# facebookresearch/habitat-lab

Measured on AMD Instinct MI355X. Metric: env-steps/sec (SPS) PointNav RGB-D 256x256, 64 envs x 128 rollout, higher is better.
Workload: dtype f32; 1 GPU; PointNav SimpleCNN+GRU, 64 envs x 128 steps, 256x256 RGB-D synthetic; envs_per_gpu=64, rollout_steps=128, ppo_epoch=4, num_mini_batch=4, parallelism=dp1

## Files before the change

habitat-lab_amd/csrc/engine.hip:

```cpp
#include <string.h>

#include <algorithm>

#include <string>
#include <vector>

#include "engine.h"

using namespace hab;

static void plan_tm_workspace(hab_policy* e, Arena& wk);
void add_tail_params(hab_policy* e) {
    const hab_policy_desc& d = e->d;
    const int H = d.hidden;
    const std::string rn = "net.state_encoder.rnn.";
    for (int l = 0; l < d.rnn_layers; ++l) {
        const int in = l == 0 ? e->rnn_in : H;
        const std::string sfx = "_l" + std::to_string(l);
        e->i_wih.push_back(add_param(e, rn + "weight_ih" + sfx, {e->G_ * H, in}));
        e->i_whh.push_back(add_param(e, rn + "weight_hh" + sfx, {e->G_ * H, H}));
        e->i_bih.push_back(add_param(e, rn + "bias_ih" + sfx, {e->G_ * H}));
        e->i_bhh.push_back(add_param(e, rn + "bias_hh" + sfx, {e->G_ * H}));
    }
    if (d.action_dist == HAB_DIST_GAUSSIAN) {
// ... 241 lines not shown
}
extern "C" int hab_policy_probe_read_tag(hab_policy* e, int tag, double* total_ms, int* count) {
    if (!e || !total_ms || !count || tag < 0 || tag >= 64) return HAB_ERR_ARG;
    return probe_sum(e, tag, total_ms, count);
}


static int encoder_forward(hab_policy* e, const hab_obs* obs, const uint8_t* masks, const int* rows, int B, hipStream_t s, int f0 = 0, int nB = -1) {
    if (e->rn) { Probe pr(e, HAB_PROBE_ENC_FWD, s); return resnet_encoder_forward(e, obs, masks, rows, B, s, f0, nB); }
    if (nB < 0) nB = B;
    float* W = e->WK;
    float* ws = W + e->w_ws;
    const int H = e->d.hidden;
    if (e->Cin == 0) {
        if (!rows && f0) return HAB_ERR_ARG;
        return gather_cols(obs->goal, e->d.goal_dim, rows ? rows + f0 : nullptr, W + e->w_rnnin + (int64_t)f0 * e->rnn_ld, e->rnn_ld, 0, e->d.goal_dim,
                           e->rnn_ld - e->rnn_in, nB, s);
    }
    const int64_t m1 = (int64_t)e->c1.Ho() * e->c1.Wo() * 32, m2 = (int64_t)e->c2.Ho() * e->c2.Wo() * 64, m3 = e->fc_in;
    float *a1 = W + e->w_a1 + f0 * m1, *a2 = W + e->w_a2 + f0 * m2, *a3 = W + e->w_a3 + f0 * m3, *rin = W + e->w_rnnin + (int64_t)f0 * e->rnn_ld;
    const int* rws = rows ? rows + f0 : nullptr;
    if (!rows && f0) return HAB_ERR_ARG;
    ObsView ov;
    ov.rgb = e->d.has_rgb ? obs->rgb : nullptr; ov.depth = e->d.has_depth ? obs->depth : nullptr; ov.rows = rws;
    ov.H = e->d.H; ov.W = e->d.W; ov.C = e->Cin;
    ConvDesc c1 = e->c1, c2 = e->c2, c3 = e->c3;
    c1.B = c2.B = c3.B = nB;
    { Probe pr(e, HAB_PROBE_CONV1_FWD, s);
      HAB_TRY(obs_conv_fwd(c1, ov, e->PK + e->pk_c1f, e->p(e->i_c1b), a1, 1, ws, e->ws_floats, s, e->pk_c1img >= 0 ? e->PK + e->pk_c1img : nullptr)); }
    { Probe pr(e, HAB_PROBE_CONV2_FWD, s);
      HAB_TRY(conv_fwd(c2, a1, e->PK + e->pk_c2f, e->p(e->i_c2b), a2, 1, ws, e->ws_floats, s)); }
    { Probe pr(e, HAB_PROBE_CONV3_FWD, s);
      HAB_TRY(conv_fwd(c3, a2, e->PK + e->pk_c3f, e->p(e->i_c3b), a3, 0, ws, e->ws_floats, s)); }
    { Probe pr(e, HAB_PROBE_FC_FWD, s);
      HAB_TRY(linear_fwd(a3, e->fc_in, e->PK + e->pk_fc, e->fc_in, e->p(e->i_fcb), rin, e->rnn_ld, nB, H, e->fc_in, 1, 0, ws, e->ws_floats, s)); }
    if (e->d.goal_dim > 0)
        HAB_TRY(gather_cols(obs->goal, e->d.goal_dim, rws, rin, e->rnn_ld, H, e->d.goal_dim, e->rnn_ld - e->rnn_in, nB, s));
    return HAB_OK;
}

static RnnForm rnn_form_cfg(const hab_policy* e, int frames, int n, bool tm_shape) {
    static const int chunks = hab_env_int("HAB_RNN_CHUNKS", 4), chunks_resnet = hab_env_int("HAB_RNN_CHUNKS_RESNET", -1);
    static const int wave = hab_env_int("HAB_RNN_WAVE", 1);
    RnnForm f;
    if (tm_shape) {
        int nc = chunks;
        if (e->rn && chunks > 1) nc = chunks_resnet >= 0 ? chunks_resnet : frames >= 4096 ? 2 : 0;
        f.chunks = std::max(0, std::min(nc, frames / n));
    }
    if (f.chunks == 0) f.wave = wave && e->L >= 2 && e->L <= 4;
    return f;
}
static RnnForm rnn_form(const hab_policy* e, const int* rows, const hab_pack_info* pack, int B, int n) {
    const bool tm_shape = e->Cin > 0 && rows && !pack->env_first_frame && (B % n) == 0 && B / n >= 2 && e->w_ws2 >= 0 &&
                          (int64_t)e->L * 2 * n <= 3 * (int64_t)e->d.max_frames;
    return rnn_form_cfg(e, B, n, tm_shape);
}
static void plan_tm_workspace(hab_policy* e, Arena& wk) {
    const int64_t B = e->d.max_frames;
    if (rnn_form_cfg(e, (int)B, 1, true).chunks == 0) return;
    e->ws2_floats = e->ws_floats;
    e->w_ws2 = wk.take(e->ws2_floats);
    e->w_fmask = wk.take((B + 3) / 4 + 64);
    e->w_iota = wk.take(B + 64);
}
static int tm_setup(hab_policy* e, int nev) {
    if (!e->s2) {
        int lo = 0, hi = 0;
        (void)hipDeviceGetStreamPriorityRange(&lo, &hi);
// ... 430 lines not shown
```

habitat-lab_amd/csrc/gemm_ops.hip:

```cpp
#include "igemm.h"
#include "igemm_dma.h"
#include "igemm_dma_wgrad.h"
#include "igemm_bf3.h"
#include "igemm_bf3_ws.h"
#include "dense_bf3.h"
#include "obs_conv_bf3.h"
#include "obs_conv_bf3_ws.h"
#include "obs_conv_patch.h"
#include "wgrad3x3_bf3.h"
#include "conv2_fwd_strip.h"
#include "conv2_dgrad_strip.h"
#include "obs_wgrad_bf3.h"
#include "conv_patch_bf3.h"
#include "wgrad3x3_patch.h"
#include "prob_build.h"
#include <stdlib.h>

#include <atomic>

#include "../../include/habitat_amd.h"

namespace hab {

static bool no_dma() { static const bool v = hab_env_flag("HAB_NO_DMA"); return v; }
static bool no_merged_dgrad() { static const bool v = hab_env_flag("HAB_NO_MERGED_DGRAD"); return v; }
static bool no_patch() { static const bool v = hab_env_flag("HAB_NO_PATCH"); return v; }
static std::atomic<int> g_bf3_mode{-1};
static int bf3_mode() {
    int m = g_bf3_mode.load(std::memory_order_relaxed);
    if (m < 0) {
        static const int from_env = hab_env_int("HAB_BF3", 2047);
        int expected = -1;
        g_bf3_mode.compare_exchange_strong(expected, from_env, std::memory_order_relaxed);
        m = g_bf3_mode.load(std::memory_order_relaxed);
    }
    return m;
}
int matrix_path_bits() { return bf3_mode(); }
extern "C" int hab_set_matrix_path(int mode) {
    const int prev = bf3_mode();
    if (mode >= 0) g_bf3_mode.store(mode, std::memory_order_relaxed);
    return prev;
}


template <class P, int TM, int TN, int WM, int WN>
static int bf3_launch(const P& p, float* ws, size_t ws_floats, int target_blocks, hipStream_t stream) {
    constexpr bool WS_SHAPE = P::A_RC && P::B_RC && TM == 2 && TN == 2 && WM == 2 && WN == 2;
    if constexpr (WS_SHAPE) {
        constexpr int ws_min_k = 2048;
        if ((bf3_mode() & 32) && p.K >= ws_min_k) return igemm_bf3_ws_launch<P, TM, TN, WM, WN, 4>(p, ws, ws_floats, target_blocks, stream);
    }
    return igemm_bf3_launch<P, TM, TN, WM, WN>(p, ws, ws_floats, target_blocks, stream);
}

template <class P>
static int run_igemm(const P& p, float* ws, size_t ws_floats, hipStream_t stream, int target_blocks = 1024) {
    if (P::A_RC || P::B_RC) target_blocks = 256;
    constexpr bool WG = !P::A_RC && !P::B_RC && AKv<P>::value == 4;
    if constexpr (P::A_RC && P::B_RC) {
        if ((bf3_mode() & 1) && p.M > 64) {
            if (p.N <= 32) return bf3_launch<P, 2, 1, 4, 1>(p, ws, ws_floats, target_blocks, stream);
            if (p.N <= 64) {
                if (p.M >= 256 * 512 && p.K >= 576) return bf3_launch<P, 2, 2, 4, 1>(p, ws, ws_floats, target_blocks, stream);
// ... 43 lines not shown
        return igemm_launch<P, 1, 2, 4, 1>(p, ws, ws_floats, target_blocks, stream);
    } else {
        if (p.M <= 64) return igemm_launch<P, 1, 2, 2, 2>(p, ws, ws_floats, target_blocks, stream);
        return igemm_launch<P, 2, 2, 2, 2>(p, ws, ws_floats, target_blocks, stream);
    }
}

int conv_fwd(const ConvDesc& d, const float* x, const float* wf, const float* bias, float* y, int relu, float* ws,
             size_t ws_floats, hipStream_t stream) {
    ConvFwdProb p;
    HAB_TRY(build(p, d, x, wf, bias, y, relu));
    if ((bf3_mode() & 256) && (bf3_mode() & 1)) {
        const int rc = conv2_fwd_strip(p, ws, ws_floats, stream);
        if (rc != 1) return rc;
    }
    if ((bf3_mode() & 16) && d.stride == 1 && d.KH == 3 && d.KW == 3 && p.M > 64) {
        PatchGeom gq{};
        gq.in = x; gq.Hi = d.H; gq.Wi = d.W; gq.Ci = d.C; gq.Ho = p.g.Ho; gq.Wo = p.g.Wo; gq.KH = 3; gq.KW = 3;
        gq.off_h = -d.pad; gq.off_w = -d.pad; gq.flip = 0;
        const int rc = conv_patch_bf3_dispatch(p, gq, ws, ws_floats, stream);
        if (rc != 1) return rc;
    }
    return run_igemm(p, ws, ws_floats, stream);
}
int64_t obs_conv_weight_image_floats() { return ((int64_t)OCP_W_ELEMS + 1) / 2 + 4; }
int obs_conv_weight_image(const float* wf, int Cout, int KH, int KW, int C, void* img, hipStream_t stream) {
    return obs_conv_patch_weight_image(wf, Cout, KH, KW, C, reinterpret_cast<unsigned short*>(img), stream);
}
int obs_conv_fwd(const ConvDesc& d, const ObsView& obs, const float* wf, const float* bias, float* y, int relu, float* ws,
                 size_t ws_floats, hipStream_t stream, const void* wimg) {
    ObsConvFwdProb p;
    HAB_TRY(build(p, d, obs, wf, bias, y, relu));
    if ((bf3_mode() & 64) && (bf3_mode() & 2) && p.quad) {
        const int rc = obs_conv_patch_launch(p, ws, ws_floats, stream, reinterpret_cast<const unsigned short*>(wimg));
        if (rc != 1) return rc;
    }
    if ((bf3_mode() & 32) && (bf3_mode() & 2) && p.quad && p.M > 64) {
        const int rc = obs_conv_bf3_ws_launch(p, ws, ws_floats, stream);
        if (rc != 1) return rc;
    }
    if ((bf3_mode() & 2) && p.quad && p.M > 64) {
        const int rc = obs_conv_bf3_launch<2>(p, ws, ws_floats, stream);
        if (rc != 1) return rc;
    }
    return run_igemm(p, ws, ws_floats, stream);
}
__global__ void dgrad_empty_class_kernel(ConvDgradProb p) {
    const long long total = (long long)p.g.B * p.Hc * p.Wc * p.N;
    for (long long e = (long long)blockIdx.x * blockDim.x + threadIdx.x; e < total; e += (long long)gridDim.x * blockDim.x)
        p.store((int)(e / p.N), (int)(e % p.N), 0.f);
}

int conv_dgrad(const ConvDesc& d, const float* dy, const float* wd, const float* mask, const float* add, float* dx,
               float* ws, size_t ws_floats, hipStream_t stream) {
    if ((bf3_mode() & 512) && (bf3_mode() & 1)) {
        const int rc = conv2_dgrad_strip(d, dy, wd, mask, add, dx, stream);
        if (rc != 1) return rc;
    }
    if (d.stride > 1 && !no_dma() && !no_merged_dgrad()) {
        ConvDgradMergedProb q;
        HAB_TRY(check_conv(d));
        q.g = make_geom(d);
        if (ConvDgradMergedProb::applicable(q.g)) {
            q.dy = dy; q.w = wd; q.mask = mask; q.add = add; q.dx = dx;
            q.finish();
            if ((bf3_mode() & 1) && q.M > 64) {
                if (q.N <= 32) return bf3_launch<ConvDgradMergedProb, 2, 1, 4, 1>(q, ws, ws_floats, 256, stream);
// ... 42 lines not shown
        ConvWgradProb q = p;
        q.colsum = nullptr;
        if (dbias) HAB_TRY(colsum(dy, p.N, p.K, p.N, dbias, 0, ws, ws_floats, stream));
        return wgrad3x3_patch(q, ws, ws_floats, stream);
    }
    if (ws && d.pad == 0 && p.N <= 32 && !no_dma() && !(bf3_mode() & 8)) {
        ConvWgradProb q = p;
        q.colsum = nullptr;
        if (wgrad_dma_ok(q)) {
            if (dbias) HAB_TRY(colsum(dy, p.N, p.K, p.N, dbias, 0, ws, ws_floats, stream));
            if ((q.M % 288 == 0) || (cdiv(q.M, 288) * 288 < cdiv(q.M, 256) * 256)) return igemm_dma_wgrad_launch<3, 3, 1>(q, ws, ws_floats, 1024, stream);
            return igemm_dma_wgrad_launch<2, 4, 1>(q, ws, ws_floats, 1024, stream);
        }
    }
    return run_igemm(p, ws, ws_floats, stream);
}
int obs_conv_wgrad(const ConvDesc& d, const ObsView& obs, const float* dy, float* dw_oihw, float* dbias, float* ws,
                   size_t ws_floats, hipStream_t stream) {
    ObsConvWgradProb p;
    HAB_TRY(build(p, d, obs, dy, dw_oihw, dbias));
    if ((bf3_mode() & 2) && p.quad && p.K > 4096) {
        const int rc = obs_wgrad_bf3_launch(p, ws, ws_floats, stream);
        if (rc != 1) return rc;
    }
    return run_igemm(p, ws, ws_floats, stream);
}
static bool dense_on() { return (bf3_mode() & 1024) && (bf3_mode() & 1); }
static bool dense_worth(long long M, long long N, long long K) {
    if (bf3_mode() & 2048) return true;
    static const long long min_flop = (long long)hab_env_int("HAB_DENSE_MIN_MFLOP", 4000) * 1000000LL;
    return 2 * M * N * K >= min_flop;
}
int linear_fwd(const float* x, int ldx, const float* w, int ldw, const float* bias, float* y, int ldy, int M, int N, int K,
               int relu, int accumulate, float* ws, size_t ws_floats, hipStream_t stream) {
    LinearFwdProb p;
    HAB_TRY(build(p, x, ldx, w, ldw, bias, y, ldy, M, N, K, relu, accumulate));
    if (dense_on() && dense_worth(M, N, K)) {
        DenseArgs g{};
        g.M = M; g.N = N; g.K = K; g.a = x; g.lda = ldx; g.b = w; g.ldb = ldw; g.c = y; g.ldc = ldy; g.bias = bias; g.relu = relu;
        g.accumulate = accumulate; g.partial = ws;
        g.a_bytes = ((long long)(M - 1) * ldx + K) * 4; g.b_bytes = ((long long)(N - 1) * ldw + K) * 4;
        if (dense_bf3_ok(g, false, false)) {
            g.nsplit = ws ? dense_bf3_splits(g, ws_floats) : 1;
            HAB_TRY((dense_bf3_launch<0, 0>(g, stream)));
            if (g.nsplit > 1) {
                igemm_splitk_reduce<LinearFwdProb>(p, ws, g.nsplit, stream);
                HAB_LAUNCH_CHECK();
            }
            return HAB_OK;
        }
    }
    return run_igemm(p, ws, ws_floats, stream);
}
int linear_dgrad(const float* dy, int lddy, const float* w, int ldw, const float* mask, int ldmask, int mask_cols, float* dx,
                 int lddx, int M, int Nin, int Kout, int accumulate, float* ws, size_t ws_floats, hipStream_t stream) {
    LinearDgradProb p;
    HAB_TRY(build(p, dy, lddy, w, ldw, mask, ldmask, mask_cols, dx, lddx, M, Nin, Kout, accumulate));
    if (dense_on() && !mask && dense_worth(M, Nin, Kout)) {
        DenseArgs g{};
        g.M = M; g.N = Nin; g.K = Kout; g.a = dy; g.lda = lddy; g.b = w; g.ldb = ldw; g.c = dx; g.ldc = lddx; g.accumulate = accumulate;
        g.partial = ws;
        g.a_bytes = ((long long)(M - 1) * lddy + Kout) * 4; g.b_bytes = ((long long)(Kout - 1) * ldw + Nin) * 4;
        if (dense_bf3_ok(g, false, true)) {
            g.nsplit = ws ? dense_bf3_splits(g, ws_floats) : 1;
            HAB_TRY((dense_bf3_launch<0, 1>(g, stream)));
            if (g.nsplit > 1) {
                igemm_splitk_reduce<LinearDgradProb>(p, ws, g.nsplit, stream);
                HAB_LAUNCH_CHECK();
            }
// ... 249 lines not shown
```

habitat-lab_amd/csrc/igemm.h:

```cpp
#pragma once
#include <type_traits>

#include "hab_common.h"

namespace hab {

constexpr int IGEMM_BK = 32;
constexpr int IGEMM_ICPAD = 4;

template <class P, class = void>
struct ColsumB : std::false_type {};
template <class P>
struct ColsumB<P, std::void_t<decltype(P::COLSUM_B)>> : std::bool_constant<P::COLSUM_B && !P::B_RC> {};

template <class P, class = void>
struct AKv : std::integral_constant<int, 4> {};
template <class P>
struct AKv<P, std::void_t<decltype(P::A_KV)>> : std::integral_constant<int, P::A_KV> {};

template <class P, class = void>
struct EpiV4 : std::false_type {};
template <class P>
struct EpiV4<P, std::void_t<decltype(P::EPI_VEC4)>> : std::bool_constant<P::EPI_VEC4> {};

template <class P, int TM, int TN>
__device__ __forceinline__ void igemm_epilogue_v4(const P& p, const f32x16 (&acc)[TM][TN], int mbase, int nbase, int li, int hi) {
    typename P::EpiCol4 ecol[TN][4];
#pragma unroll
    for (int j = 0; j < TN; ++j)
#pragma unroll
        for (int g = 0; g < 4; ++g) ecol[j][g] = p.epi_col4(nbase + j * 32 + 8 * g + 4 * hi);
#pragma unroll
    for (int i = 0; i < TM; ++i) {
        const typename P::EpiRow erow = p.epi_row(mbase + i * 32 + li);
#pragma unroll
        for (int j = 0; j < TN; ++j) {
            typename P::EpiAux4 aux[4];
#pragma unroll
            for (int g = 0; g < 4; ++g) aux[g] = p.epi_fetch4(erow, ecol[j][g]);
#pragma unroll
            for (int g = 0; g < 4; ++g) {
                f32x4 v;
                v[0] = acc[i][j][4 * g]; v[1] = acc[i][j][4 * g + 1]; v[2] = acc[i][j][4 * g + 2]; v[3] = acc[i][j][4 * g + 3];
                p.epi_store4(erow, ecol[j][g], aux[g], v);
            }
        }
    }
}

template <class P, int TM, int TN>
__device__ __forceinline__ void igemm_partial_v4(const P& p, const f32x16 (&acc)[TM][TN], float* __restrict__ slab, int mbase, int nbase,
                                                 int li, int hi) {
    const bool vec = ((p.N & 3) == 0) && ((reinterpret_cast<uintptr_t>(slab) & 15) == 0);
#pragma unroll
    for (int i = 0; i < TM; ++i) {
        const int row = mbase + i * 32 + li;
// ... 234 lines not shown
#pragma unroll
        for (int g = 0; g < 4; ++g) {
            typename P::EpiRow erow[4];
            typename P::EpiAux eaux[4][TN];
#pragma unroll
            for (int q = 0; q < 4; ++q) {
                erow[q] = p.epi_row(m0 + (wm * TM + i) * 32 + q + 8 * g + 4 * hi);
#pragma unroll
                for (int j = 0; j < TN; ++j) eaux[q][j] = p.epi_fetch(erow[q], ecol[j]);
            }
#pragma unroll
            for (int q = 0; q < 4; ++q)
#pragma unroll
                for (int j = 0; j < TN; ++j) p.epi_store(erow[q], ecol[j], eaux[q][j], acc[i][j][g * 4 + q]);
        }
}

template <class P, bool WIDE>
__global__ void __launch_bounds__(256) igemm_splitk_reduce_kernel(const P p, const float* __restrict__ partial, int splits) {
    __shared__ float red[4][64];
    int MP = p.M;
    if constexpr (ColsumB<P>::value) MP += (p.colsum != nullptr) ? 1 : 0;
    const size_t total = (size_t)MP * p.N;
    if constexpr (!WIDE) {
        for (size_t e = (size_t)blockIdx.x * 256 + threadIdx.x; e < total; e += (size_t)gridDim.x * 256) {
            float s = 0.0f;
            for (int z = 0; z < splits; ++z) s += partial[(size_t)z * total + e];
            const int m = (int)(e / p.N), n = (int)(e % p.N);
            if constexpr (ColsumB<P>::value) {
                if (m == p.M) { p.store_colsum(n, s); continue; }
            }
            p.store(m, n, s);
        }
        return;
    }
    const int tx = threadIdx.x & 63, ty = threadIdx.x >> 6;
    const int chunk = (splits + 3) >> 2;
    const int z0 = ty * chunk, z1 = min(splits, z0 + chunk);
    for (size_t e0 = (size_t)blockIdx.x * 64; e0 < total; e0 += (size_t)gridDim.x * 64) {
        const size_t e = e0 + tx;
        float s = 0.0f;
        if (e < total) {
            const float* src = partial + e;
            int z = z0;
            for (; z + 8 <= z1; z += 8) {
                float v[8];
#pragma unroll
                for (int u = 0; u < 8; ++u) v[u] = src[(size_t)(z + u) * total];
#pragma unroll
                for (int u = 0; u < 8; ++u) s += v[u];
            }
            for (; z < z1; ++z) s += src[(size_t)z * total];
        }
        red[ty][tx] = s;
        __syncthreads();
        if (ty == 0 && e < total) {
            s = (red[0][tx] + red[1][tx]) + (red[2][tx] + red[3][tx]);
            const int m = (int)(e / p.N), n = (int)(e % p.N);
            bool done = false;
            if constexpr (ColsumB<P>::value) {
                if (m == p.M) { p.store_colsum(n, s); done = true; }
            }
            if (!done) p.store(m, n, s);
        }
        __syncthreads();
    }
}

template <class P>
inline void igemm_splitk_reduce(const P& p, const float* ws, int splits, hipStream_t stream) {
    const long long total = (long long)(p.M + 1) * p.N;
    if (splits >= 16) {
        int blocks = (int)cdivl(total, 64);
        if (blocks > 8192) blocks = 8192;
        igemm_splitk_reduce_kernel<P, true><<<blocks, 256, 0, stream>>>(p, ws, splits);
    } else {
        int blocks = (int)cdivl(total, 256);
        if (blocks > 4096) blocks = 4096;
        igemm_splitk_reduce_kernel<P, false><<<blocks, 256, 0, stream>>>(p, ws, splits);
    }
}

struct IgemmPlan {
    int splits = 1;
    int k_per_split = 0;
    size_t partial_floats = 0;
};

inline IgemmPlan igemm_plan(int BM, int BN, int M, int N, int K, int target_blocks, int max_splits, size_t max_partial_floats) {
    IgemmPlan pl;
    const long long tiles = (long long)cdiv(M, BM) * cdiv(N, BN);
    int splits = 1;
    if (tiles < target_blocks) splits = (int)((target_blocks + tiles - 1) / tiles);
    const int ktiles = cdiv(K, IGEMM_BK);
    if (splits > ktiles) splits = ktiles;
    if (splits > max_splits) splits = max_splits;
    while (splits > 1 && (size_t)splits * (size_t)(M + 1) * (size_t)N > max_partial_floats) --splits;
    if (splits < 1) splits = 1;
    pl.k_per_split = cdiv(ktiles, splits) * IGEMM_BK;
    pl.splits = cdiv(K, pl.k_per_split);
    pl.partial_floats = pl.splits > 1 ? (size_t)pl.splits * (M + 1) * N : 0;
    return pl;
}

// ... 20 lines not shown
```

habitat-lab_amd/csrc/obs_conv_patch.h:

```cpp
#pragma once
#include <utility>

#include "igemm_bf3.h"

namespace hab {

constexpr int OCP_TH = 4;
constexpr int OCP_R = 4 * OCP_TH + 4;
constexpr int OCP_KP = 256 + 8;
constexpr int OCP_DP = 64 + 8;

constexpr int OCP_W_ELEMS = 3 * 32 * OCP_KP + 2 * 32 * OCP_DP;
__global__ void obs_patch_split_weights(const float* __restrict__ w, int N, unsigned short* __restrict__ img) {
    const int e = blockIdx.x * blockDim.x + threadIdx.x;
    if (e >= 32 * 256) return;
    const int n = e >> 8, k = e & 255, c = k & 3;
    float v = n < N ? w[(size_t)n * 256 + k] : 0.f;
    if (c < 3) v *= HAB_RCP255;
    unsigned h1, h2, h3;
    bf3_split(v, h1, h2, h3);
    img[(0 * 32 + n) * OCP_KP + k] = (unsigned short)h1;
    img[(1 * 32 + n) * OCP_KP + k] = (unsigned short)h2;
    img[(2 * 32 + n) * OCP_KP + k] = (unsigned short)h3;
    if (c == 3) {
        unsigned short* d = img + 3 * 32 * OCP_KP;
        const int kd = k >> 2;
        d[(0 * 32 + n) * OCP_DP + kd] = (unsigned short)h1;
        d[(1 * 32 + n) * OCP_DP + kd] = (unsigned short)h2;
    }
    if (k < 8) {
        img[(0 * 32 + n) * OCP_KP + 256 + k] = 0; img[(1 * 32 + n) * OCP_KP + 256 + k] = 0; img[(2 * 32 + n) * OCP_KP + 256 + k] = 0;
        unsigned short* d = img + 3 * 32 * OCP_KP;
        d[(0 * 32 + n) * OCP_DP + 64 + k] = 0; d[(1 * 32 + n) * OCP_DP + 64 + k] = 0;
    }
}

template <class F, int... Is>
__device__ __forceinline__ void ocp_static_for_impl(F& f, std::integer_sequence<int, Is...>) { (f(std::integral_constant<int, Is>()), ...); }
template <int N, class F>
__device__ __forceinline__ void ocp_static_for(F& f) { ocp_static_for_impl(f, std::make_integer_sequence<int, N>()); }

struct ObsPatchGeom {
    int W, H, Ho, Wo, tiles_per_img, ntiles;
    int units;
    int patch_elems;
};

template <int UPT>
__global__ void __launch_bounds__(512) obs_conv_patch_kernel(const ObsConvFwdProb p, const ObsPatchGeom gq, const unsigned short* __restrict__ wimg,
                                                              const int sign_schedule, const int ablate) {
    using P = ObsConvFwdProb;
    static_assert(EpiV4<P>::value, "transposed-accumulator epilogue");
    extern __shared__ __attribute__((aligned(16))) unsigned short smem16[];
    const int W = gq.W;
    const int t = threadIdx.x;
    const int lane = t & 63, wave = __builtin_amdgcn_readfirstlane(t >> 6), group = wave >> 2, gw = wave & 3, tg = t & 255;
    const int li = lane & 31, hi = lane >> 5;
    unsigned short* W12 = smem16;
    unsigned short* WD1 = W12 + 2 * 32 * OCP_KP;
    float* biasL = reinterpret_cast<float*>(WD1 + 32 * OCP_DP);
    unsigned short* P0 = WD1 + 32 * OCP_DP + 64 + group * gq.patch_elems;
    unsigned short* P1 = P0 + OCP_R * W * 4;
    unsigned short* P2 = P1 + OCP_R * W;

    for (int i = t; i < 2 * 32 * OCP_KP / 8; i += 512) reinterpret_cast<u32x4*>(W12)[i] = reinterpret_cast<const u32x4*>(wimg)[i];
    for (int i = t; i < 32 * OCP_DP / 8; i += 512) reinterpret_cast<u32x4*>(WD1)[i] = reinterpret_cast<const u32x4*>(wimg + 3 * 32 * OCP_KP)[i];
    if (t < 32) biasL[t] = (p.bias && t < p.N) ? p.bias[t] : 0.f;
    bf16x8 w3f[8][2], wd2f[4];
    {
        const unsigned short* w3 = wimg + 2 * 32 * OCP_KP + li * OCP_KP + hi * 8;
        const unsigned short* wd = wimg + 3 * 32 * OCP_KP + li * OCP_DP + hi * 8;
#pragma unroll
        for (int kh = 0; kh < 8; ++kh)
#pragma unroll
            for (int s = 0; s < 2; ++s) w3f[kh][s] = *reinterpret_cast<const bf16x8*>(w3 + kh * 32 + s * 16);
#pragma unroll
        for (int j = 0; j < 4; ++j) wd2f[j] = *reinterpret_cast<const bf16x8*>(wd + 32 * OCP_DP + j * 16);
    }

    auto tile_of = [&](int vb) {
        const int q = gq.ntiles >> 3, r = gq.ntiles & 7, xcd = vb & 7, idx = vb >> 3;
// ... 10 lines not shown
        return (size_t)p.obs.srow(img) * gq.H;
    };
    auto unit_pix = [&](size_t frame, int y0, int j, bool& ok) {
        const int u = tg + 256 * j;
        const int r = u / qpr, x4 = u - r * qpr;
        const int y = y0 + r;
        ok = (u < gq.units) & (y < gq.H);
        return (frame + (ok ? y : 0)) * W + 4 * (ok ? x4 : 0);
    };
    auto fetch_depth = [&](int tile) {
        if (ablate & 1) return;
        int y0;
        const size_t frame = tile_base(tile, y0);
#pragma unroll
        for (int j = 0; j < UPT; ++j) {
            bool ok;
            const size_t pix = unit_pix(frame, y0, j, ok);
            dp[j] = ld4(p.obs.depth + pix);
            if (!ok) dp[j] = zero4();
        }
    };
    auto fetch_rgb = [&](int tile) {
        if (ablate & 1) return;
        int y0;
        const size_t frame = tile_base(tile, y0);
#pragma unroll
        for (int j = 0; j < UPT; ++j) {
            bool ok;
            const size_t pix = unit_pix(frame, y0, j, ok);
            rg[j] = *reinterpret_cast<const Rgb12*>(p.obs.rgb + pix * 3);
            if (!ok) { rg[j].d0 = 0; rg[j].d1 = 0; rg[j].d2 = 0; }
        }
    };
    auto stage = [&]() {
        if (ablate & 8) return;
#pragma unroll
        for (int j = 0; j < UPT; ++j) {
            const int u = tg + 256 * j;
            if (u >= gq.units) continue;
            const unsigned d[3] = {rg[j].d0, rg[j].d1, rg[j].d2};
            unsigned f[12];
#pragma unroll
            for (int e = 0; e < 12; ++e) f[e] = __float_as_uint((float)((d[e >> 2] >> (8 * (e & 3))) & 0xffu));
            unsigned a1, a2, a3, b1, b2, b3;
            bf3_split2(dp[j][0], dp[j][1], a1, a2, a3);
            bf3_split2(dp[j][2], dp[j][3], b1, b2, b3);
            u32x4 lo, hi4;
            lo[0] = bf3_pack(f[0], f[1]);  lo[1] = bf3_pack(f[2], a1 << 16);
            lo[2] = bf3_pack(f[3], f[4]);  lo[3] = bf3_pack(f[5], a1 & 0xffff0000u);
            hi4[0] = bf3_pack(f[6], f[7]); hi4[1] = bf3_pack(f[8], b1 << 16);
            hi4[2] = bf3_pack(f[9], f[10]); hi4[3] = bf3_pack(f[11], b1 & 0xffff0000u);
            unsigned short* dst = P0 + (size_t)u * 16;
            *reinterpret_cast<u32x4*>(dst) = lo;
            *reinterpret_cast<u32x4*>(dst + 8) = hi4;
            u32x2 r1, r2;
            r1[0] = a2; r1[1] = b2; r2[0] = a3; r2[1] = b3;
            *reinterpret_cast<u32x2*>(P1 + (size_t)u * 4) = r1;
            *reinterpret_cast<u32x2*>(P2 + (size_t)u * 4) = r2;
        }
    };

    const int a_px0 = (4 * gw) * W + 4 * li;
    f32x16 acc[2];
    bf16x8 fr[2][5];
    auto load_step = [&](auto stc) {
        constexpr int st = decltype(stc)::value, set = st & 1;
        if constexpr (st < 4) {
#pragma unroll
            for (int i = 0; i < 2; ++i) {
                const int px = a_px0 + (2 * st + hi) * W + 128 * i;
                u32x4 v1, v2;
                const u32x2 l1 = *reinterpret_cast<const u32x2*>(P1 + px), h1 = *reinterpret_cast<const u32x2*>(P1 + px + 4);
                const u32x2 l2 = *reinterpret_cast<const u32x2*>(P2 + px), h2 = *reinterpret_cast<const u32x2*>(P2 + px + 4);
                v1[0] = l1[0]; v1[1] = l1[1]; v1[2] = h1[0]; v1[3] = h1[1];
                v2[0] = l2[0]; v2[1] = l2[1]; v2[2] = h2[0]; v2[3] = h2[1];
                fr[set][i] = __builtin_bit_cast(bf16x8, v1);
                fr[set][2 + i] = __builtin_bit_cast(bf16x8, v2);
            }
            fr[set][4] = *reinterpret_cast<const bf16x8*>(WD1 + li * OCP_DP + (2 * st + hi) * 8);
        } else {
            constexpr int kh = (st - 4) >> 1, s_ = (st - 4) & 1;
#pragma unroll
            for (int i = 0; i < 2; ++i)
                fr[set][i] = *reinterpret_cast<const bf16x8*>(P0 + (size_t)(a_px0 + kh * W + 128 * i) * 4 + (2 * s_ + hi) * 8);
#pragma unroll
            for (int pl = 0; pl < 2; ++pl)
                fr[set][2 + pl] = *reinterpret_cast<const bf16x8*>(W12 + (pl * 32 + li) * OCP_KP + kh * 32 + s_ * 16 + hi * 8);
        }
    };
    auto flip = [&](bf16x8 f, const unsigned sgn) {
        u32x4 v = __builtin_bit_cast(u32x4, f);
        v[0] ^= sgn; v[1] ^= sgn; v[2] ^= sgn; v[3] ^= sgn;
        return __builtin_bit_cast(bf16x8, v);
    };
    auto mma_step = [&](auto stc, const unsigned sgn) {
        constexpr int st = decltype(stc)::value, set = st & 1;
        if constexpr (st < 4) {
            const bf16x8 a1[2] = {flip(fr[set][0], sgn), flip(fr[set][1], sgn)}, a2[2] = {flip(fr[set][2], sgn), flip(fr[set][3], sgn)};
            const bf16x8 wd1 = fr[set][4];
#pragma unroll
            for (int i = 0; i < 2; ++i) acc[i] = __builtin_amdgcn_mfma_f32_32x32x16_bf16(wd1, a2[i], acc[i], 0, 0, 0);
#pragma unroll
            for (int i = 0; i < 2; ++i) acc[i] = __builtin_amdgcn_mfma_f32_32x32x16_bf16(wd2f[st], a1[i], acc[i], 0, 0, 0);
#pragma unroll
            for (int i = 0; i < 2; ++i) acc[i] = __builtin_amdgcn_mfma_f32_32x32x16_bf16(wd1, a1[i], acc[i], 0, 0, 0);
        } else {
            constexpr int kh = (st - 4) >> 1, s_ = (st - 4) & 1;
            const bf16x8 a[2] = {flip(fr[set][0], sgn), flip(fr[set][1], sgn)};
#pragma unroll
            for (int i = 0; i < 2; ++i) acc[i] = __builtin_amdgcn_mfma_f32_32x32x16_bf16(w3f[kh][s_], a[i], acc[i], 0, 0, 0);
#pragma unroll
            for (int i = 0; i < 2; ++i) acc[i] = __builtin_amdgcn_mfma_f32_32x32x16_bf16(fr[set][3], a[i], acc[i], 0, 0, 0);
#pragma unroll
            for (int i = 0; i < 2; ++i) acc[i] = __builtin_amdgcn_mfma_f32_32x32x16_bf16(fr[set][2], a[i], acc[i], 0, 0, 0);
        }
    };
    auto matrix_phase = [&](const unsigned sgn) {
#pragma unroll
        for (int i = 0; i < 2; ++i)
#pragma unroll
            for (int v = 0; v < 16; ++v) acc[i][v] = 0.0f;
        if (ablate & 2) return;
        load_step(std::integral_constant<int, 0>());
// ... 3 lines not shown
            mma_step(stc, sgn);
        };
        ocp_static_for<20>(body);
    };
    auto store_tile = [&](int tile, bool neg) {
        if ((ablate & 4) && acc[0][0] != 12345.f) return;
        const int img = tile / gq.tiles_per_img, ho = (tile - img * gq.tiles_per_img) * OCP_TH + gw;
        if (ho >= gq.Ho) return;
#pragma unroll
        for (int i = 0; i < 2; ++i) {
            const int wo = 32 * i + li;
            if (wo >= gq.Wo) continue;
            const size_t base = ((size_t)(img * gq.Ho + ho) * gq.Wo + wo) * p.N;
#pragma unroll
            for (int g = 0; g < 4; ++g) {
                const int n = 8 * g + 4 * hi;
                if (n + 3 >= p.N) continue;
                f32x4 v;
                v[0] = acc[i][4 * g]; v[1] = acc[i][4 * g + 1]; v[2] = acc[i][4 * g + 2]; v[3] = acc[i][4 * g + 3];
                if (neg) { v[0] = -v[0]; v[1] = -v[1]; v[2] = -v[2]; v[3] = -v[3]; }
                v += *reinterpret_cast<const f32x4*>(biasL + n);
                if (p.relu) { v[0] = fmaxf(v[0], 0.f); v[1] = fmaxf(v[1], 0.f); v[2] = fmaxf(v[2], 0.f); v[3] = fmaxf(v[3], 0.f); }
                if (p.y) *reinterpret_cast<f32x4*>(p.y + base + n) = v;
            }
        }
    };

    const int vstep = 2 * gridDim.x;
    const int vb0 = blockIdx.x + group * gridDim.x;
    const int n_mine = vb0 < gq.ntiles ? (gq.ntiles - vb0 + vstep - 1) / vstep : 0;
    const int n_first = (int)blockIdx.x < gq.ntiles ? (gq.ntiles - (int)blockIdx.x + vstep - 1) / vstep : 0;
    if (n_first == 0) return;
    if (n_mine > 0) { fetch_depth(tile_of(vb0)); if (group == 0) fetch_rgb(tile_of(vb0)); }
    if (group == 0) stage();
    __syncthreads();
    for (int pI = 0; pI <= 2 * n_first; ++pI) {
        if ((pI & 1) == group) {
            const int k = pI >> 1;
            if (k < n_mine) {
                if (k + 1 < n_mine) fetch_depth(tile_of(vb0 + (k + 1) * vstep));
                const int tile = tile_of(vb0 + k * vstep);
                matrix_phase((sign_schedule && (tile & 1)) ? 0x80008000u : 0u);
            }
        } else {
            const int kd = (pI - 1 - group) / 2;
            const int ks = (pI + 1 - group) / 2;
            if (ks < n_mine) {
                fetch_rgb(tile_of(vb0 + ks * vstep));
                stage();
            }
            if (pI >= 1 + group && kd < n_mine) {
                const int tile_d = tile_of(vb0 + kd * vstep);
                store_tile(tile_d, sign_schedule && (tile_d & 1));
            }
        }
        __syncthreads();
    }
}

inline int obs_conv_patch_weight_image(const float* w_packed, int N, int KH, int KW, int C, unsigned short* img, hipStream_t stream) {
    if (KH != 8 || KW != 8 || C != 4 || N > 32 || (N & 3) || !w_packed || !img || (reinterpret_cast<uintptr_t>(img) & 15)) return 1;
    obs_patch_split_weights<<<32, 256, 0, stream>>>(w_packed, N, img);
    HAB_LAUNCH_CHECK();
    return HAB_OK;
}

inline int obs_conv_patch_launch(const ObsConvFwdProb& p, float* ws, size_t ws_floats, hipStream_t stream, const unsigned short* wimg_cached = nullptr) {
    const ConvGeom& g = p.g;
    if (!p.quad || g.KH != 8 || g.KW != 8 || g.stride != 4 || g.pad != 0 || p.N > 32 || (p.N & 3) || p.K != 256 || g.W > 256 || (g.W & 3) || g.Wo > 64 ||
        g.Wo < 1 || p.M <= 0)
        return 1;
    if (!wimg_cached && (!ws || ws_floats * 4 < (size_t)OCP_W_ELEMS * 2 || (reinterpret_cast<uintptr_t>(ws) & 15))) return 1;
    if (reinterpret_cast<uintptr_t>(wimg_cached) & 15) return 1;
    ObsPatchGeom gq;
    gq.W = g.W; gq.H = g.H; gq.Ho = g.Ho; gq.Wo = g.Wo;
    gq.tiles_per_img = cdiv(g.Ho, OCP_TH);
    gq.ntiles = g.B * gq.tiles_per_img;
    gq.units = OCP_R * (g.W >> 2);
    if (cdiv(gq.units, 256) > 5) return 1;
    gq.patch_elems = OCP_R * g.W * 6 + 64;
    const size_t lds = ((size_t)2 * 32 * OCP_KP + 32 * OCP_DP + 64 + (size_t)2 * gq.patch_elems) * 2;
    if (lds > 160 * 1024) return 1;
    const unsigned short* wimg = wimg_cached;
    if (!wimg) {
        unsigned short* built = reinterpret_cast<unsigned short*>(ws);
        obs_patch_split_weights<<<32, 256, 0, stream>>>(p.w, p.N, built);
        HAB_LAUNCH_CHECK();
        wimg = built;
    }
    auto kern = obs_conv_patch_kernel<5>;
    static const hipError_t attr_err = hipFuncSetAttribute(reinterpret_cast<const void*>(kern), hipFuncAttributeMaxDynamicSharedMemorySize, 160 * 1024);
    if (attr_err != hipSuccess) return (int)attr_err;
    static const int sign_schedule = !hab_env_flag("HAB_BF3_NOSIGN");
    static const int ablate = hab_env_int("HAB_OCP_ABLATE", 0);
    const int pairs = (gq.ntiles + 1) / 2;
    const int grid = pairs < 256 ? (pairs + 7) / 8 * 8 : 256;
    kern<<<grid, 512, lds, stream>>>(p, gq, wimg, sign_schedule, ablate);
    HAB_LAUNCH_CHECK();
    return HAB_OK;
}

}
```

habitat-lab_amd/csrc/ops.h:

```cpp
#pragma once
#include "hab_common.h"

namespace hab {

struct ConvDesc {
    int B, H, W, C, Cout, KH, KW, stride, pad;
    int Creal = 0;
    int Ho() const { return (H + 2 * pad - KH) / stride + 1; }
    int Wo() const { return (W + 2 * pad - KW) / stride + 1; }
};
struct ObsView;

int conv_fwd(const ConvDesc& d, const float* x, const float* wf, const float* bias, float* y, int relu, float* ws,
             size_t ws_floats, hipStream_t stream);
int obs_conv_fwd(const ConvDesc& d, const ObsView& obs, const float* wf, const float* bias, float* y, int relu, float* ws,
                 size_t ws_floats, hipStream_t stream, const void* wimg = nullptr);
int64_t obs_conv_weight_image_floats();
int obs_conv_weight_image(const float* wf, int Cout, int KH, int KW, int C, void* img, hipStream_t stream);
int conv_dgrad(const ConvDesc& d, const float* dy, const float* wd, const float* mask, const float* add, float* dx,
               float* ws, size_t ws_floats, hipStream_t stream);
int conv_wgrad(const ConvDesc& d, const float* x, const float* dy, float* dw_oihw, float* dbias, float* ws, size_t ws_floats,
               hipStream_t stream);
int obs_conv_wgrad(const ConvDesc& d, const ObsView& obs, const float* dy, float* dw_oihw, float* dbias, float* ws,
                   size_t ws_floats, hipStream_t stream);
int linear_fwd(const float* x, int ldx, const float* w, int ldw, const float* bias, float* y, int ldy, int M, int N, int K,
               int relu, int accumulate, float* ws, size_t ws_floats, hipStream_t stream);
int linear_dgrad(const float* dy, int lddy, const float* w, int ldw, const float* mask, int ldmask, int mask_cols, float* dx,
                 int lddx, int M, int Nin, int Kout, int accumulate, float* ws, size_t ws_floats, hipStream_t stream);
int linear_wgrad(const float* dy, int lddy, const float* x, int ldx, float* dw, int lddw, int Mrows, int Nout, int Kin,
                 int perm_c, int perm_hw, int accumulate, float* ws, size_t ws_floats, hipStream_t stream);
int colsum(const float* a, int lda, int M, int N, float* out, int accumulate, float* ws, size_t ws_floats, hipStream_t stream);
int repack_conv(const float* w_oihw, float* wf, float* wd, int Cout, int Cin, int KH, int KW, int cpad, hipStream_t stream);
int repack_flatten(const float* w, float* wp, int N, int C, int HW, hipStream_t stream);
int transpose2d(const float* w, float* wt, int R, int C, hipStream_t stream);
int pad_rows(const float* w, float* wp, int R, int C, int ld, hipStream_t stream);

struct PackInfo {
    const int* select_inds;
    const int* step_offsets;
    const int* num_seqs_at_step;
    const int* frag_env;
    const int* frag_start;
    int P, F, max_len, n_envs;
};

struct RnnLayerParams {
    const float* w_ih; const float* w_hh; const float* b_ih; const float* b_hh;
    const float* w_hh_t;
    float* dw_ih; float* dw_hh; float* db_ih; float* db_hh;
    int in_dim;
    const float* w_ih_pad = nullptr;
    int w_ih_ld = 0;
};

struct RnnWork {
    float* gi;
    float* gates;
    float* hn;
    float* hprev;
// ... 39 lines not shown
```

habitat-lab_amd/csrc/prob_build.h:

```cpp
#pragma once
#include "ops.h"
#include "problems.h"

namespace hab {

inline ConvGeom make_geom(const ConvDesc& d) {
    ConvGeom g;
    g.B = d.B; g.H = d.H; g.W = d.W; g.C = d.C; g.Cout = d.Cout; g.KH = d.KH; g.KW = d.KW; g.stride = d.stride; g.pad = d.pad;
    g.finish();
    return g;
}

inline int check_conv(const ConvDesc& d) {
    if (d.B <= 0 || d.H <= 0 || d.W <= 0 || d.C <= 0 || d.Cout <= 0 || d.KH <= 0 || d.KW <= 0 || d.stride <= 0 || d.pad < 0)
        return HAB_ERR_ARG;
    if ((long long)d.B * d.H * d.W >= (1ll << 31)) return HAB_ERR_UNSUPPORTED;
    if ((d.H + 2 * d.pad - d.KH) < 0 || (d.W + 2 * d.pad - d.KW) < 0) return HAB_ERR_ARG;
    return HAB_OK;
}

inline bool aligned16(const void* p) { return (((uintptr_t)p) & 15) == 0; }

inline int obs_quad_ok(const ConvDesc& d, const ObsView& obs) {
    return obs.rgb && obs.depth && obs.C == 4 && d.KW % 4 == 0 && d.stride % 4 == 0 && d.pad == 0 && d.W % 4 == 0 &&
// ... 19 lines not shown
}
inline int build(ConvDgradProb& p, const ConvDesc& d, const float* dy, const float* wd, const float* mask, const float* add,
                 float* dx, int ph = 0, int pw = 0) {
    HAB_TRY(check_conv(d));
    if (d.C % 4 || d.Cout % 4) return HAB_ERR_UNSUPPORTED;
    if (ph < 0 || pw < 0 || ph >= d.stride || pw >= d.stride) return HAB_ERR_ARG;
    p.g = make_geom(d);
    p.dy = dy; p.w = wd; p.mask = mask; p.add = add; p.dx = dx;
    p.set_class(ph, pw);
    return HAB_OK;
}
inline int build(ConvWgradProb& p, const ConvDesc& d, const float* x, const float* dy, float* dw, float* dbias = nullptr) {
    HAB_TRY(check_conv(d));
    if (d.C % 4 || d.Cout % 4) return HAB_ERR_UNSUPPORTED;
    p.g = make_geom(d);
    p.M = d.KH * d.KW * d.C; p.N = d.Cout; p.K = d.B * p.g.Ho * p.g.Wo;
    p.x = x; p.dy = dy; p.dw = dw; p.colsum = dbias;
    p.Creal = d.Creal > 0 ? d.Creal : d.C;
    return HAB_OK;
}
inline int build(ObsConvWgradProb& p, const ConvDesc& d, const ObsView& obs, const float* dy, float* dw, float* dbias = nullptr) {
    HAB_TRY(check_conv(d));
    if (d.C != obs.C || d.Cout % 4) return HAB_ERR_UNSUPPORTED;
    p.g = make_geom(d);
    p.M = d.KH * d.KW * d.C; p.N = d.Cout; p.K = d.B * p.g.Ho * p.g.Wo;
    p.obs = obs; p.dy = dy; p.dw = dw; p.colsum = dbias;
    p.quad = obs_quad_ok(d, obs);
    return HAB_OK;
}
inline int build(LinearFwdProb& p, const float* x, int ldx, const float* w, int ldw, const float* bias, float* y, int ldy,
                 int M, int N, int K, int relu, int accumulate) {
    if (M <= 0 || N <= 0 || K <= 0 || !x || !w || !y) return HAB_ERR_ARG;
    p.M = M; p.N = N; p.K = K; p.x = x; p.ldx = ldx; p.w = w; p.ldw = ldw; p.bias = bias; p.y = y; p.ldy = ldy;
    p.relu = relu; p.accumulate = accumulate;
    p.vec = (ldx % 4 == 0 && ldw % 4 == 0 && K % 4 == 0 && aligned16(x) && aligned16(w)) ? 1 : 0;
    return HAB_OK;
}
inline int build(LinearDgradProb& p, const float* dy, int lddy, const float* w, int ldw, const float* mask, int ldmask,
                 int mask_cols, float* dx, int lddx, int M, int Nin, int Kout, int accumulate) {
    if (M <= 0 || Nin <= 0 || Kout <= 0 || !dy || !w || !dx) return HAB_ERR_ARG;
    if (!aligned16(w)) return HAB_ERR_ARG;
    p.M = M; p.N = Nin; p.K = Kout; p.dy = dy; p.lddy = lddy; p.w = w; p.ldw = ldw; p.mask = mask; p.ldmask = ldmask;
    p.mask_cols = mask_cols; p.dx = dx; p.lddx = lddx; p.accumulate = accumulate;
    p.vec_a = (lddy % 4 == 0 && Kout % 4 == 0 && aligned16(dy)) ? 1 : 0;
    return HAB_OK;
}
inline int build(LinearWgradProb& p, const float* dy, int lddy, const float* x, int ldx, float* dw, int lddw, int Mrows,
                 int Nout, int Kin, int perm_c, int perm_hw, int accumulate) {
    if (Mrows <= 0 || Nout <= 0 || Kin <= 0 || !dy || !x || !dw) return HAB_ERR_ARG;
    if (!aligned16(dy) || !aligned16(x)) return HAB_ERR_ARG;
    p.M = Nout; p.N = Kin; p.K = Mrows; p.dy = dy; p.lddy = lddy; p.x = x; p.ldx = ldx; p.dw = dw; p.lddw = lddw;
    p.perm_c = perm_c; p.perm_hw = perm_hw; p.dPermC = FastDiv(perm_c > 0 ? perm_c : 1); p.accumulate = accumulate;
    return HAB_OK;
}

}
```

habitat-lab_amd/csrc/problems.h:

```cpp
#pragma once
#include <math.h>

#include "hab_common.h"
#include "bf3_split.h"

namespace hab {

#define HAB_HD __host__ __device__ inline

HAB_HD f32x4 zero4() {
    f32x4 z;
    z[0] = 0.f; z[1] = 0.f; z[2] = 0.f; z[3] = 0.f;
    return z;
}
HAB_HD f32x4 ld4(const float* p) { return *reinterpret_cast<const f32x4*>(p); }

struct Raw4 { f32x4 v; int ok; };
struct KKey { int k, ok; };
HAB_HD KKey kkey(int k, int k_end) { KKey q; q.k = k; q.ok = k < k_end; return q; }
HAB_HD f32x4 sel4(const Raw4& r) { return r.ok ? r.v : zero4(); }
struct NoCtx {};
struct NoAux {};

constexpr int HAB_FAR = -(1 << 28);
// ... 874 lines not shown
        if (!(r.ok & c.ok)) return;
        dw[(size_t)c.n * g.C * g.KH * g.KW + r.off] = v * r.scale;
    }
    HAB_GENERIC_STORE
};

HAB_HD Raw4 row_fetch4(const float* row, int row_ok, const KKey& q, int K, int vec) {
    Raw4 r;
    if (vec) {
        r.ok = row_ok & q.ok;
        r.v = ld4(row + (q.k & -r.ok));
    } else {
        r.ok = 1;
        r.v = zero4();
        for (int e = 0; e < 4; ++e)
            if (row_ok && q.ok && q.k + e < K) r.v[e] = row[q.k + e];
    }
    return r;
}
HAB_HD Raw4 col_fetch4(const float* base, int ld, int r, int r_ok, int j, int n) {
    Raw4 q;
    if (((ld & 3) == 0) && (j + 3 < n || j >= n)) {
        q.ok = r_ok & (j < n);
        q.v = ld4(base + (((size_t)r * ld + j) & (size_t)(-(long long)q.ok)));
    } else {
        q.ok = 1;
        q.v = zero4();
        for (int e = 0; e < 4; ++e)
            if (r_ok && j + e < n) q.v[e] = base[(size_t)r * ld + j + e];
    }
    return q;
}

struct LinearFwdProb {
    static constexpr bool A_RC = true, B_RC = true;
    int M, N, K;
    const float* x; int ldx;
    const float* w; int ldw;
    const float* bias;
    float* y; int ldy;
    int relu, vec;
    int accumulate;
    HAB_NO_KCTX
    using ACtx = WRowCtx;
    using BCtx = WRowCtx;
    using ARaw = Raw4;
    using BRaw = Raw4;
    HAB_HD ACtx a_ctx(int m) const { ACtx c; c.ok = m < M; c.row = c.ok ? x + (size_t)m * ldx : x; return c; }
    using AKey = KKey;
    using BKey = KKey;
    HAB_HD AKey a_key(const KCtx&, int k, int k_end) const { return kkey(k, k_end); }
    HAB_HD BKey b_key(const KCtx&, int k, int k_end) const { return kkey(k, k_end); }
    HAB_HD ARaw a_fetch(const ACtx& c, const KCtx&, const AKey& q) const { return row_fetch4(c.row, c.ok, q, K, vec); }
    HAB_HD BCtx b_ctx(int n) const { BCtx c; c.ok = n < N; c.row = c.ok ? w + (size_t)n * ldw : w; return c; }
    HAB_HD BRaw b_fetch(const BCtx& c, const KCtx&, const BKey& q) const { return row_fetch4(c.row, c.ok, q, K, vec); }
    HAB_PLAIN_CVT
    using EpiCol = ColN;
    using EpiRow = RowBase;
    struct EpiAux { float old; };
    HAB_HD EpiCol epi_col(int n) const { EpiCol c; c.n = n; c.ok = n < N; c.bias = (bias && c.ok) ? bias[n] : 0.f; return c; }
    HAB_HD EpiRow epi_row(int m) const { EpiRow r; r.ok = m < M; r.base = (size_t)m * ldy; return r; }
    HAB_HD EpiAux epi_fetch(const EpiRow& r, const EpiCol& c) const {
        EpiAux a;
        a.old = accumulate ? y[(r.ok & c.ok) ? r.base + c.n : 0] : 0.f;
        return a;
    }
    HAB_HD void epi_store(const EpiRow& r, const EpiCol& c, const EpiAux& a, float v) const {
        if (!(r.ok & c.ok)) return;
        v += c.bias;
        v += a.old;
        if (relu) v = v > 0.f ? v : 0.f;
        y[r.base + c.n] = v;
    }
    HAB_GENERIC_STORE
};
// ... 98 lines not shown
```

Measured before the change: 62990 env-steps/s.

## Fuse goal-column gather into FC split-K reduce and pre-sign staged obs patches

The goal-vector gather into the RNN input buffer is folded into the split-K reduce epilogue of the FC linear forward, which removes a separate gather_cols launch whenever that path runs. Separately, the obs conv1 patch kernel gets a template variant that applies the alternating-tile sign flip while staging to LDS rather than on every fragment in the matrix phase. Both are enabled by default through new HAB_BF3 bits. The tail write only fires on the split-K path and otherwise falls back to the old gather via a host-side written flag, and it adds a strided scalar loop to the reduce kernel.

```diff
diff --git a/habitat-lab_amd/csrc/engine.hip b/habitat-lab_amd/csrc/engine.hip
--- a/habitat-lab_amd/csrc/engine.hip
+++ b/habitat-lab_amd/csrc/engine.hip
@@ -297,9 +297,14 @@
       HAB_TRY(conv_fwd(c2, a1, e->PK + e->pk_c2f, e->p(e->i_c2b), a2, 1, ws, e->ws_floats, s)); }
     { Probe pr(e, HAB_PROBE_CONV3_FWD, s);
       HAB_TRY(conv_fwd(c3, a2, e->PK + e->pk_c3f, e->p(e->i_c3b), a3, 0, ws, e->ws_floats, s)); }
+    int goal_written = 0;
+    ColsTail goal;
+    goal.src = obs->goal; goal.src_ld = e->d.goal_dim; goal.rows = rws; goal.col0 = H; goal.ncols = e->d.goal_dim; goal.npad = e->rnn_ld - e->rnn_in;
+    goal.written = &goal_written;
     { Probe pr(e, HAB_PROBE_FC_FWD, s);
-      HAB_TRY(linear_fwd(a3, e->fc_in, e->PK + e->pk_fc, e->fc_in, e->p(e->i_fcb), rin, e->rnn_ld, nB, H, e->fc_in, 1, 0, ws, e->ws_floats, s)); }
-    if (e->d.goal_dim > 0)
+      HAB_TRY(linear_fwd(a3, e->fc_in, e->PK + e->pk_fc, e->fc_in, e->p(e->i_fcb), rin, e->rnn_ld, nB, H, e->fc_in, 1, 0, ws, e->ws_floats, s,
+                         (e->d.goal_dim > 0 && obs->goal) ? &goal : nullptr)); }
+    if (e->d.goal_dim > 0 && !goal_written)
         HAB_TRY(gather_cols(obs->goal, e->d.goal_dim, rws, rin, e->rnn_ld, H, e->d.goal_dim, e->rnn_ld - e->rnn_in, nB, s));
     return HAB_OK;
 }
diff --git a/habitat-lab_amd/csrc/gemm_ops.hip b/habitat-lab_amd/csrc/gemm_ops.hip
--- a/habitat-lab_amd/csrc/gemm_ops.hip
+++ b/habitat-lab_amd/csrc/gemm_ops.hip
@@ -29,7 +29,7 @@
 static int bf3_mode() {
     int m = g_bf3_mode.load(std::memory_order_relaxed);
     if (m < 0) {
-        static const int from_env = hab_env_int("HAB_BF3", 2047);
+        static const int from_env = hab_env_int("HAB_BF3", 2047 | 8192 | 16384);
         int expected = -1;
         g_bf3_mode.compare_exchange_strong(expected, from_env, std::memory_order_relaxed);
         m = g_bf3_mode.load(std::memory_order_relaxed);
@@ -139,7 +139,7 @@
     ObsConvFwdProb p;
     HAB_TRY(build(p, d, obs, wf, bias, y, relu));
     if ((bf3_mode() & 64) && (bf3_mode() & 2) && p.quad) {
-        const int rc = obs_conv_patch_launch(p, ws, ws_floats, stream, reinterpret_cast<const unsigned short*>(wimg));
+        const int rc = obs_conv_patch_launch(p, ws, ws_floats, stream, reinterpret_cast<const unsigned short*>(wimg), (bf3_mode() & 16384) != 0);
         if (rc != 1) return rc;
     }
     if ((bf3_mode() & 32) && (bf3_mode() & 2) && p.quad && p.M > 64) {
@@ -248,9 +248,10 @@
     return 2 * M * N * K >= min_flop;
 }
 int linear_fwd(const float* x, int ldx, const float* w, int ldw, const float* bias, float* y, int ldy, int M, int N, int K,
-               int relu, int accumulate, float* ws, size_t ws_floats, hipStream_t stream) {
+               int relu, int accumulate, float* ws, size_t ws_floats, hipStream_t stream, const ColsTail* tail) {
     LinearFwdProb p;
     HAB_TRY(build(p, x, ldx, w, ldw, bias, y, ldy, M, N, K, relu, accumulate));
+    if (tail && (bf3_mode() & 8192)) p.tail = *tail;
     if (dense_on() && dense_worth(M, N, K)) {
         DenseArgs g{};
         g.M = M; g.N = N; g.K = K; g.a = x; g.lda = ldx; g.b = w; g.ldb = ldw; g.c = y; g.ldc = ldy; g.bias = bias; g.relu = relu;
diff --git a/habitat-lab_amd/csrc/igemm.h b/habitat-lab_amd/csrc/igemm.h
--- a/habitat-lab_amd/csrc/igemm.h
+++ b/habitat-lab_amd/csrc/igemm.h
@@ -22,6 +22,11 @@
 struct EpiV4 : std::false_type {};
 template <class P>
 struct EpiV4<P, std::void_t<decltype(P::EPI_VEC4)>> : std::bool_constant<P::EPI_VEC4> {};
+
+template <class P, class = void>
+struct SplitkTail : std::false_type {};
+template <class P>
+struct SplitkTail<P, std::void_t<decltype(P::SPLITK_TAIL)>> : std::bool_constant<P::SPLITK_TAIL> {};
 
 template <class P, int TM, int TN>
 __device__ __forceinline__ void igemm_epilogue_v4(const P& p, const f32x16 (&acc)[TM][TN], int mbase, int nbase, int li, int hi) {
@@ -322,6 +327,7 @@
             }
             p.store(m, n, s);
         }
+        if constexpr (SplitkTail<P>::value) p.store_tail((int)(blockIdx.x * 256 + threadIdx.x), (int)(gridDim.x * 256));
         return;
     }
     const int tx = threadIdx.x & 63, ty = threadIdx.x >> 6;
@@ -355,11 +361,15 @@
         }
         __syncthreads();
     }
+    if constexpr (SplitkTail<P>::value) p.store_tail((int)(blockIdx.x * 256 + threadIdx.x), (int)(gridDim.x * 256));
 }
 
 template <class P>
 inline void igemm_splitk_reduce(const P& p, const float* ws, int splits, hipStream_t stream) {
     const long long total = (long long)(p.M + 1) * p.N;
+    if constexpr (SplitkTail<P>::value) {
+        if (p.tail.src && p.tail.written) *p.tail.written = 1;
+    }
     if (splits >= 16) {
         int blocks = (int)cdivl(total, 64);
         if (blocks > 8192) blocks = 8192;
diff --git a/habitat-lab_amd/csrc/obs_conv_patch.h b/habitat-lab_amd/csrc/obs_conv_patch.h
--- a/habitat-lab_amd/csrc/obs_conv_patch.h
+++ b/habitat-lab_amd/csrc/obs_conv_patch.h
@@ -46,7 +46,7 @@
     int patch_elems;
 };
 
-template <int UPT>
+template <int UPT, bool STAGE_SIGN>
 __global__ void __launch_bounds__(512) obs_conv_patch_kernel(const ObsConvFwdProb p, const ObsPatchGeom gq, const unsigned short* __restrict__ wimg,
                                                               const int sign_schedule, const int ablate) {
     using P = ObsConvFwdProb;
@@ -123,7 +123,7 @@
             if (!ok) { rg[j].d0 = 0; rg[j].d1 = 0; rg[j].d2 = 0; }
         }
     };
-    auto stage = [&]() {
+    auto stage = [&](const unsigned sgn) {
         if (ablate & 8) return;
 #pragma unroll
         for (int j = 0; j < UPT; ++j) {
@@ -141,11 +141,16 @@
             lo[2] = bf3_pack(f[3], f[4]);  lo[3] = bf3_pack(f[5], a1 & 0xffff0000u);
             hi4[0] = bf3_pack(f[6], f[7]); hi4[1] = bf3_pack(f[8], b1 << 16);
             hi4[2] = bf3_pack(f[9], f[10]); hi4[3] = bf3_pack(f[11], b1 & 0xffff0000u);
+            u32x2 r1, r2;
+            r1[0] = a2; r1[1] = b2; r2[0] = a3; r2[1] = b3;
+            if constexpr (STAGE_SIGN) {
+#pragma unroll
+                for (int q = 0; q < 4; ++q) { lo[q] ^= sgn; hi4[q] ^= sgn; }
+                r1[0] ^= sgn; r1[1] ^= sgn; r2[0] ^= sgn; r2[1] ^= sgn;
+            }
             unsigned short* dst = P0 + (size_t)u * 16;
             *reinterpret_cast<u32x4*>(dst) = lo;
             *reinterpret_cast<u32x4*>(dst + 8) = hi4;
-            u32x2 r1, r2;
-            r1[0] = a2; r1[1] = b2; r2[0] = a3; r2[1] = b3;
             *reinterpret_cast<u32x2*>(P1 + (size_t)u * 4) = r1;
             *reinterpret_cast<u32x2*>(P2 + (size_t)u * 4) = r2;
         }
@@ -180,6 +185,7 @@
         }
     };
     auto flip = [&](bf16x8 f, const unsigned sgn) {
+        if constexpr (STAGE_SIGN) return f;
         u32x4 v = __builtin_bit_cast(u32x4, f);
         v[0] ^= sgn; v[1] ^= sgn; v[2] ^= sgn; v[3] ^= sgn;
         return __builtin_bit_cast(bf16x8, v);
@@ -249,7 +255,8 @@
     const int n_first = (int)blockIdx.x < gq.ntiles ? (gq.ntiles - (int)blockIdx.x + vstep - 1) / vstep : 0;
     if (n_first == 0) return;
     if (n_mine > 0) { fetch_depth(tile_of(vb0)); if (group == 0) fetch_rgb(tile_of(vb0)); }
-    if (group == 0) stage();
+    auto tile_sgn = [&](int tile) { return (sign_schedule && (tile & 1)) ? 0x80008000u : 0u; };
+    if (group == 0) stage(n_mine > 0 ? tile_sgn(tile_of(vb0)) : 0u);
     __syncthreads();
     for (int pI = 0; pI <= 2 * n_first; ++pI) {
         if ((pI & 1) == group) {
@@ -257,14 +264,15 @@
             if (k < n_mine) {
                 if (k + 1 < n_mine) fetch_depth(tile_of(vb0 + (k + 1) * vstep));
                 const int tile = tile_of(vb0 + k * vstep);
-                matrix_phase((sign_schedule && (tile & 1)) ? 0x80008000u : 0u);
+                matrix_phase(tile_sgn(tile));
             }
         } else {
             const int kd = (pI - 1 - group) / 2;
             const int ks = (pI + 1 - group) / 2;
             if (ks < n_mine) {
-                fetch_rgb(tile_of(vb0 + ks * vstep));
-                stage();
+                const int tile_s = tile_of(vb0 + ks * vstep);
+                fetch_rgb(tile_s);
+                stage(tile_sgn(tile_s));
             }
             if (pI >= 1 + group && kd < n_mine) {
                 const int tile_d = tile_of(vb0 + kd * vstep);
@@ -282,7 +290,8 @@
     return HAB_OK;
 }
 
-inline int obs_conv_patch_launch(const ObsConvFwdProb& p, float* ws, size_t ws_floats, hipStream_t stream, const unsigned short* wimg_cached = nullptr) {
+inline int obs_conv_patch_launch(const ObsConvFwdProb& p, float* ws, size_t ws_floats, hipStream_t stream, const unsigned short* wimg_cached = nullptr,
+                                 bool stage_sign = true) {
     const ConvGeom& g = p.g;
     if (!p.quad || g.KH != 8 || g.KW != 8 || g.stride != 4 || g.pad != 0 || p.N > 32 || (p.N & 3) || p.K != 256 || g.W > 256 || (g.W & 3) || g.Wo > 64 ||
         g.Wo < 1 || p.M <= 0)
@@ -305,14 +314,16 @@
         HAB_LAUNCH_CHECK();
         wimg = built;
     }
-    auto kern = obs_conv_patch_kernel<5>;
-    static const hipError_t attr_err = hipFuncSetAttribute(reinterpret_cast<const void*>(kern), hipFuncAttributeMaxDynamicSharedMemorySize, 160 * 1024);
+    static const hipError_t attr_err = hipFuncSetAttribute(reinterpret_cast<const void*>(obs_conv_patch_kernel<5, false>), hipFuncAttributeMaxDynamicSharedMemorySize, 160 * 1024);
     if (attr_err != hipSuccess) return (int)attr_err;
+    static const hipError_t attr_err_s = hipFuncSetAttribute(reinterpret_cast<const void*>(obs_conv_patch_kernel<5, true>), hipFuncAttributeMaxDynamicSharedMemorySize, 160 * 1024);
+    if (attr_err_s != hipSuccess) return (int)attr_err_s;
     static const int sign_schedule = !hab_env_flag("HAB_BF3_NOSIGN");
     static const int ablate = hab_env_int("HAB_OCP_ABLATE", 0);
     const int pairs = (gq.ntiles + 1) / 2;
     const int grid = pairs < 256 ? (pairs + 7) / 8 * 8 : 256;
-    kern<<<grid, 512, lds, stream>>>(p, gq, wimg, sign_schedule, ablate);
+    if (stage_sign) obs_conv_patch_kernel<5, true><<<grid, 512, lds, stream>>>(p, gq, wimg, sign_schedule, ablate);
+    else obs_conv_patch_kernel<5, false><<<grid, 512, lds, stream>>>(p, gq, wimg, sign_schedule, ablate);
     HAB_LAUNCH_CHECK();
     return HAB_OK;
 }
diff --git a/habitat-lab_amd/csrc/ops.h b/habitat-lab_amd/csrc/ops.h
--- a/habitat-lab_amd/csrc/ops.h
+++ b/habitat-lab_amd/csrc/ops.h
@@ -23,8 +23,9 @@
                hipStream_t stream);
 int obs_conv_wgrad(const ConvDesc& d, const ObsView& obs, const float* dy, float* dw_oihw, float* dbias, float* ws,
                    size_t ws_floats, hipStream_t stream);
+struct ColsTail;
 int linear_fwd(const float* x, int ldx, const float* w, int ldw, const float* bias, float* y, int ldy, int M, int N, int K,
-               int relu, int accumulate, float* ws, size_t ws_floats, hipStream_t stream);
+               int relu, int accumulate, float* ws, size_t ws_floats, hipStream_t stream, const ColsTail* tail = nullptr);
 int linear_dgrad(const float* dy, int lddy, const float* w, int ldw, const float* mask, int ldmask, int mask_cols, float* dx,
                  int lddx, int M, int Nin, int Kout, int accumulate, float* ws, size_t ws_floats, hipStream_t stream);
 int linear_wgrad(const float* dy, int lddy, const float* x, int ldx, float* dw, int lddw, int Mrows, int Nout, int Kin,
diff --git a/habitat-lab_amd/csrc/prob_build.h b/habitat-lab_amd/csrc/prob_build.h
--- a/habitat-lab_amd/csrc/prob_build.h
+++ b/habitat-lab_amd/csrc/prob_build.h
@@ -75,7 +75,7 @@
                  int M, int N, int K, int relu, int accumulate) {
     if (M <= 0 || N <= 0 || K <= 0 || !x || !w || !y) return HAB_ERR_ARG;
     p.M = M; p.N = N; p.K = K; p.x = x; p.ldx = ldx; p.w = w; p.ldw = ldw; p.bias = bias; p.y = y; p.ldy = ldy;
-    p.relu = relu; p.accumulate = accumulate;
+    p.relu = relu; p.accumulate = accumulate; p.tail = ColsTail();
     p.vec = (ldx % 4 == 0 && ldw % 4 == 0 && K % 4 == 0 && aligned16(x) && aligned16(w)) ? 1 : 0;
     return HAB_OK;
 }
diff --git a/habitat-lab_amd/csrc/problems.h b/habitat-lab_amd/csrc/problems.h
--- a/habitat-lab_amd/csrc/problems.h
+++ b/habitat-lab_amd/csrc/problems.h
@@ -930,8 +930,16 @@
     return q;
 }
 
+struct ColsTail {
+    const float* src = nullptr; int src_ld = 0;
+    const int* rows = nullptr;
+    int col0 = 0, ncols = 0, npad = 0;
+    int* written = nullptr;
+};
+
 struct LinearFwdProb {
     static constexpr bool A_RC = true, B_RC = true;
+    static constexpr bool SPLITK_TAIL = true;
     int M, N, K;
     const float* x; int ldx;
     const float* w; int ldw;
@@ -939,6 +947,15 @@
     float* y; int ldy;
     int relu, vec;
     int accumulate;
+    ColsTail tail;
+    HAB_HD void store_tail(int e0, int stride) const {
+        if (!tail.src) return;
+        const int per = tail.ncols + tail.npad;
+        for (int e = e0; e < M * per; e += stride) {
+            const int f = e / per, c = e % per;
+            y[(size_t)f * ldy + tail.col0 + c] = (c < tail.ncols) ? tail.src[(size_t)(tail.rows ? tail.rows[f] : f) * tail.src_ld + c] : 0.f;
+        }
+    }
     HAB_NO_KCTX
     using ACtx = WRowCtx;
     using BCtx = WRowCtx;
```

Result: no change. 62950 env-steps/s (-0.1%).
